# elybrand/quantized_neural_networks

Measured on AMD Instinct MI355X. Metric: weights_quantized_per_sec, higher is better.
Workload: dtype f64; 1 GPU; Dense(4096->4096) whole-layer GPFQ, m=1024 calibration samples, M=3 alphabet, alphabet_scalar=3 (BASELINE.json configs[1], the north-star layer); N=4096, C=4096, m=1024, M=3, neurons_per_gpu=4096, arithmetic=f32 products / f64 residual and dot products (reference's mixed flow)

## Files before the change

### quantized_neural_networks_amd/csrc/gpfq_blk.hip

```cpp
#include <atomic>
#include <cmath>
#include <cstring>
#include <type_traits>

#include <cstdlib>
#include <mutex>
#include "gpfq_device.hpp"
#include <hip/hip_ext.h>
#include "gpfq_launch.hpp"
#include "gpfq_roles.hpp"

namespace gpfq {

namespace {

struct BlkStats {
    double rden, G, cb, ca, Ea, nrm;
    double sE1, sE2;
};
struct BandEntry {
    double H1, H2, E1, E2;
};
static_assert(sizeof(BlkStats) == 64 && sizeof(BandEntry) == 32, "header layout");

// ... 433 lines not shown
template <int S, int NSW> struct BlkSplit { static constexpr const int *pw = PairSplit<S>::pw; };
template <> struct BlkSplit<4, 4>   { static constexpr int pw_[4] = {1, 1, 1, 1}; static constexpr const int *pw = pw_; };
template <> struct BlkSplit<32, 11> { static constexpr int pw_[11] = {3, 3, 3, 3, 3, 3, 3, 2, 3, 3, 3}; static constexpr const int *pw = pw_; };
template <> struct BlkSplit<24, 11> { static constexpr int pw_[11] = {2, 2, 2, 2, 2, 2, 2, 1, 3, 3, 3}; static constexpr const int *pw = pw_; };

template <> struct BlkSplit<64, 11> { static constexpr int pw_[11] = {4, 6, 6, 6, 6, 6, 6, 6, 6, 6, 6}; static constexpr const int *pw = pw_; };
template <> struct BlkSplit<48, 11> { static constexpr int pw_[11] = {4, 5, 4, 4, 5, 4, 4, 5, 4, 4, 5}; static constexpr const int *pw = pw_; };
template <> struct BlkSplit<16, 11> { static constexpr int pw_[11] = {2, 2, 1, 1, 2, 2, 1, 1, 1, 1, 2}; static constexpr const int *pw = pw_; };

struct BlkSplitQuad32 { static constexpr int pw[8] = {2, 5, 5, 4, 2, 5, 5, 4}; };
struct BlkSplitFour16 { static constexpr int pw[8] = {1, 2, 2, 3, 2, 2, 2, 2}; };
template <int S> struct BlkSplit7;
template <> struct BlkSplit7<32> { static constexpr int pw[7] = {5, 5, 5, 2, 5, 5, 5}; };
template <> struct BlkSplit7<24> { static constexpr int pw[7] = {4, 4, 4, 1, 4, 4, 3}; };
template <> struct BlkSplit7<16> { static constexpr int pw[7] = {3, 3, 2, 1, 3, 2, 2}; };
template <int G, int S, int NSW, int NL> constexpr const int *blk_split()
{
    if constexpr (NSW == 7) return BlkSplit7<S>::pw;
    else
    if constexpr (G == 4 && NL < 4 && S == 32 && NSW == 8) return BlkSplitQuad32::pw;
    else if constexpr (G == 1 && NL == 4 && S == 16 && NSW == 8) return BlkSplitFour16::pw;
    else return BlkSplit<S, NSW>::pw;
}

template <int G, int S, int NSW, int NL> constexpr bool blk_split_has(int k)
{
    for (int w = 0; w < NSW; ++w)
        if (blk_split<G, S, NSW, NL>()[w] == k) return true;
    return false;
}

template <int G, int PW, int MP, int B, int NSW, bool SYM, int NL, int CLM>
// ... 1 lines not shown
{
    constexpr bool CL = CLM != 0;
    constexpr int NB = NL * G, KQ = 64 / G, NW = blk_slots(NSW, NB);
    constexpr int RSH = NL == 4 ? 0 : (NL == 2 ? 1 : 2);
    constexpr int HDR = blk_hdr_bytes(B, CL);
    constexpr int RB = (int)blk_rec_bytes(MP, B, G, CL);
    lchar *lds = (lchar *)lds_generic;
    const int ng = lane & (G - 1), kq = lane / G, row = lane >> 4;
    const bool writer = (lane & 15 & ~(G - 1)) == 0 && (row & ((1 << RSH) - 1)) == 0;
    const int nloc = NL * ng;
    const int nrow = row >> RSH;
    const int64_t jbase = cs.cl * NB;
    const unsigned ldsT_addr = lds_addr(lds_generic), ldsW_addr = lds_addr(lds_generic + L.off_w);
    const int64_t N = K.N;
    const int nslots = K.nblk + 1;
    const int o_x  = HDR + 8 * (pbase + kq);
    int o_q = o_x + 4 * MP;
    asm volatile("" : "+v"(o_q));
    constexpr int DB = blk_row64(G, B) ? 16 : 8;
    const int o_d  = HDR + 8 * MP + DB * (pbase + kq);
    using DRaw = std::conditional_t<blk_row64(G, B), double2, float2>;
    auto ld_d = [&](int off) -> DRaw { return lds_ld<DRaw>(lds, off); };
    auto to_d2 = [](const DRaw &v) -> double2 { return make_double2((double)v.x, (double)v.y); };
    const int o_wq = L.off_wq + nloc * B * 8;
    const int o_dw = L.off_d + (wave * B * NB + nloc + nrow) * 8;
    const int o_x2 = L.off_x2 + (wave * NB + nloc + nrow) * 16;

    double u[NL][2 * PW];
#pragma unroll
    for (int i = 0; i < NL; ++i)
#pragma unroll
        for (int e = 0; e < 2 * PW; ++e) u[i][e] = 0.0;

    constexpr int NPIECES = (B * RB + 1023) >> 10;
    constexpr int PER_MIN = NPIECES / NSW;
// ... 18 lines not shown
    constexpr int NHP = (B * HDR + 1023) >> 10;
    auto load_headers = [&](int b2, int buf) {
        if (wave < NHP && b2 <= K.nblk)
            glds16_s(K.hdrs + (int64_t)b2 * B * HDR + ((int64_t)wave << 10), lane16,
                     lds_addr(lds_generic + L.off_hr) + (unsigned)buf * (unsigned)L.hr_pitch + ((unsigned)wave << 10));
    };
    for (int k = 0; wave + NSW * k < NPIECES; ++k) issue_piece(0, k);
    load_weights(0);
    load_headers(0, 0); load_headers(1, 1);
    dma_wait();
    slot_barrier();
    int hbuf = 2;
    unsigned long long st0 = 0, st1 = 0, st2 = 0, st3 = 0, st4 = 0, st5 = 0, acc_dma = 0, acc_u = 0, acc_d = 0, acc_w = 0, acc_b = 0, acc_t = 0;
    (void)st0; (void)st1; (void)st2; (void)st3; (void)st4; (void)st5; (void)acc_dma; (void)acc_u; (void)acc_d; (void)acc_w; (void)acc_b; (void)acc_t;

    constexpr bool kMfmaD = G == 4 && B == 4 && blk_row64(G, B) && !kNoMfmaD;
    constexpr bool kFused = kMfmaD && !kNoFused;
    constexpr bool kBatchTop = kFused && NL == 4 && NSW == 11;
    constexpr bool kTopSym = kBatchTop && SYM;
    constexpr bool kLateHdr = kTopSym && PW >= 2 && (kTop3 & 1) != 0, kLateW = kTopSym && PW >= 2 && (kTop3 & 2) != 0;
    constexpr int kHdrStep = PW >= 3 ? 8 : 6, kWStep = PW >= 3 ? 10 : 7;
    static_assert(!(kLateHdr || kLateW) || (PW <= 3 && B == 4 && PTS == 2 && PER_MIN <= 6), "the free pair-steps of a two- or three-pair wavefront");
    static_assert(!kLateW || NB * B == 64, "one 256-byte weight piece per block");
    unsigned long long w_lanes = 0ull, w_tail = 0ull;
    int w_whole = 0;
    const float *wsrc = nullptr;
    if constexpr (kLateW) {
        w_lanes = wave == 0 ? __builtin_amdgcn_ballot_w64(jbase + lane / B < K.C) : 0ull;
        w_tail = w_lanes & (0x1111111111111111ull * ((1ull << (int)(N % B)) - 1ull));
        w_whole = (int)(N / B);
        wsrc = K.Wt + (jbase + lane / B) * K.ldw + (int64_t)(B + lane % B) * K.ldt;
    }
    (void)w_lanes; (void)w_tail; (void)w_whole; (void)wsrc;
    constexpr bool kPreloadAll = PW * B <= 8 && PW <= 5 && !kFused;
    constexpr bool kHoist = kPreloadAll && PW * B <= 4;
    constexpr int PB = kPreloadAll ? B : 1, PP = kPreloadAll ? PW : 1;
    constexpr bool kPreD = kHoist && PW * B * (blk_row64(G, B) ? 4 : 2) <= 16 && !kMfmaD;
// ... 27 lines not shown
            const int nb_ = ((b + 1) & 1) * L.tile_pitch;
            const int cbq = (b & 1) * NB * B * 8;
            double eu[NL], ew[NL];
#pragma unroll
            for (int n = 0; n < NL; ++n) { eu[n] = 0.0; ew[n] = 0.0; }
#pragma unroll
            for (int n = 0; n < NL; ++n) {
                const float w = lds_ld<float2>(lds, o_wq + cbq + (n * B + S) * 8).x;
#pragma unroll 1
                for (int p = 0; p < PW; ++p) {
                    double t0 = u[n][0], t1 = u[n][1];
#pragma unroll
                    for (int pp = 1; pp < PW; ++pp) { t0 = (p == pp) ? u[n][2 * pp] : t0; t1 = (p == pp) ? u[n][2 * pp + 1] : t1; }
                    for (int j = 0; j < S; ++j) {
                        const int rb = nb_ + j * RB;
                        const float2 x2 = lds_ld<float2>(lds, rb + o_x + 8 * p * KQ), q2 = lds_ld<float2>(lds, rb + o_q + 8 * p * KQ);
                        const float2 wq = lds_ld<float2>(lds, o_wq + cbq + (n * B + j) * 8);
                        if constexpr (SYM) {
                            t0 += (double)__fmaf_rn(wq.y, q2.x, __fmul_rn(wq.x, x2.x));
                            t1 += (double)__fmaf_rn(wq.y, q2.y, __fmul_rn(wq.x, x2.y));
                        } else {
                            t0 += (double)__fsub_rn(__fmul_rn(wq.x, x2.x), __fmul_rn(wq.y, q2.x));
                            t1 += (double)__fsub_rn(__fmul_rn(wq.x, x2.y), __fmul_rn(wq.y, q2.y));
                        }
                    }
                    const int rb = nb_ + S * RB;
                    const float2 x2 = lds_ld<float2>(lds, rb + o_x + 8 * p * KQ);
                    float2 q2;
                    if constexpr (SYM) {
                        const int i0 = 2 * (pbase + p * KQ + kq);
                        const float *xr = K.Xq + ((int64_t)b * B + S) * K.ldx + (CL ? (int64_t)cs.slice * MP : (int64_t)0);
                        const int mrow = CL ? cs.m_sl : K.m;
                        q2.x = i0 < mrow ? xr[i0] : 0.f;
                        q2.y = i0 + 1 < mrow ? xr[i0 + 1] : 0.f;
                    } else {
                        q2 = lds_ld<float2>(lds, rb + o_q + 8 * p * KQ);
                    }
                    eu[n] = fma((double)q2.x, t0, eu[n]);
                    eu[n] = fma((double)q2.y, t1, eu[n]);
                    ew[n] = fma((double)q2.x, t0 + (double)__fmul_rn(w, x2.x), ew[n]);
                    ew[n] = fma((double)q2.y, t1 + (double)__fmul_rn(w, x2.y), ew[n]);
                }
            }
            const double vu = fold_klanes_n<G, NL>(eu), vw = fold_klanes_n<G, NL>(ew);
            if (writer) lds_st<double2>(lds, o_x2, make_double2(vu, vw));
            slot_barrier();
            slot_barrier();
            if constexpr (kBatchTop) ctl = lds_read_now(lds + L.off_ctl + 4 * (b & 1));
            else ctl = lds_ld<int>(lds, L.off_ctl + 4 * (b & 1));
        }
    };
// ... 27 lines not shown
            for (int n = 0; n < NL; ++n) pr[n] = pk2{wv[n], wv[n]} * xv;
            if constexpr (SYM) {
#pragma unroll
                for (int n = 0; n < NL; ++n) dd[n] = __builtin_elementwise_fma(pk2{qv[n], qv[n]}, qx, pr[n]);
            } else {
#pragma unroll
                for (int n = 0; n < NL; ++n) rr[n] = pk2{qv[n], qv[n]} * qx;
#pragma unroll
                for (int n = 0; n < NL; ++n) dd[n] = pr[n] - rr[n];
            }
#pragma unroll
            for (int n = 0; n < NL; ++n) { c0[n] = (double)dd[n].x; c1[n] = (double)dd[n].y; }
#pragma unroll
            for (int n = 0; n < NL; ++n) { u[n][2 * p] += c0[n]; u[n][2 * p + 1] += c1[n]; }
        };
        if constexpr (kFused) {
            const int rbm = tbase + ng * RB + o_d;
            constexpr int PF = NSW == 7 ? 2 : 1, NPS = PW * B;
            float2 fwq[B][NL], xbuf[PF], qbuf[PF];
            double2 dcur;
            auto row_off = [&](int i, bool q) { return tbase + (i % B) * RB + (q ? o_q : o_x) + 8 * (i / B) * KQ; };
            auto first_requests = [&]() {
#pragma unroll
                for (int s = 0; s < B; ++s)
#pragma unroll
                    for (int n = 0; n < NL; ++n) fwq[s][n] = lds_ld<float2>(lds, o_wq + pbq + (n * B + s) * 8);
#pragma unroll
                for (int i = 0; i < PF; ++i)
                    if (i < NPS) { xbuf[i] = lds_ld<float2>(lds, row_off(i, false)); qbuf[i] = lds_ld<float2>(lds, row_off(i, true)); }
                dcur = lds_ld<double2>(lds, rbm);
            };
            if constexpr (kTopSym) {
                static_assert(!kTopSym || (B == 4 && NL == 4 && PF == 1), "slot_top_sym: four neurons per lane, pair-steps 0..2 are pair 0's steps 0..2");
                nf4 w01[4], w23[4];
                nf2 x2n, q2n;
                nd2 d0;
                __builtin_amdgcn_s_setprio(2);
                slot_top_sym<RB>(w01, w23, x2n, q2n, d0, u[0][0], u[0][1], u[1][0], u[1][1], u[2][0], u[2][1], u[3][0], u[3][1],
                                 lds + row_off(0, false), lds + row_off(0, true), lds + o_wq + pbq, lds + rbm);
                __builtin_amdgcn_s_waitcnt(0xC07F);
                xbuf[0] = make_float2(x2n.x, x2n.y); qbuf[0] = make_float2(q2n.x, q2n.y);
                dcur = make_double2(d0.x, d0.y);
#pragma unroll
                for (int n = 0; n < NL; ++n) {
                    fwq[0][n] = make_float2(w01[n].x, w01[n].y); fwq[1][n] = make_float2(w01[n].z, w01[n].w);
                    fwq[2][n] = make_float2(w23[n].x, w23[n].y); fwq[3][n] = make_float2(w23[n].z, w23[n].w);
                }
// ... 1 lines not shown
                static_assert(!kBatchTop || (B == 4 && NL == 4), "lds_read_slot_top reads four neurons' steps 0 and 1: 16 bytes at a stride of 4 steps x 8 bytes");
                nf2 x0, q0;
                nf4 w01[4];
                lds_read_slot_top(x0, q0, w01, lds + row_off(0, false), lds + row_off(0, true), lds + o_wq + pbq);
                xbuf[0] = make_float2(x0.x, x0.y); qbuf[0] = make_float2(q0.x, q0.y);
#pragma unroll
                for (int n = 0; n < NL; ++n) { fwq[0][n] = make_float2(w01[n].x, w01[n].y); fwq[1][n] = make_float2(w01[n].z, w01[n].w); }
#pragma unroll
                for (int s = 2; s < B; ++s)
#pragma unroll
                    for (int n = 0; n < NL; ++n) fwq[s][n] = lds_ld<float2>(lds, o_wq + pbq + (n * B + s) * 8);
                dcur = lds_ld<double2>(lds, rbm);
            } else {
                first_requests();
            }
            double2 dprev = make_double2(0.0, 0.0);
            double acc[NL];
#pragma unroll
            for (int n = 0; n < NL; ++n) acc[n] = 0.0;
            auto mfma_pair = [&](int pp, int i, const double2 &dd) {
                const int n = i % NL, e = i / NL;
                acc[n] = __builtin_amdgcn_mfma_f64_4x4x4f64(u[n][2 * pp + e], e ? dd.y : dd.x, acc[n], 0, 0, 0);
            };
#pragma unroll
            for (int p = 0; p < PW; ++p) {
                {
                    const int pr = 2 - (3 * p) / PW;
                    if (p == 0 || pr != 2 - (3 * (p - 1)) / PW) {
                        const int v = pr;
                        if (v >= 2) __builtin_amdgcn_s_setprio(2);
                        else if (v == 1) __builtin_amdgcn_s_setprio(1);
                        else __builtin_amdgcn_s_setprio(0);
                    }
                }
                if (p > 0) dcur = lds_ld<double2>(lds, rbm + DB * p * KQ);
#pragma unroll
                for (int st = 0; st < B; ++st) {
                    const int ips = p * B + st;
                    if (kTopSym && ips < 2) continue;
                    const float2 x2 = xbuf[ips % PF], q2 = qbuf[ips % PF];
                    const int pn = (ips + 1) / B, sn = (ips + 1) % B;
                    (void)pn; (void)sn;
                    if (ips + PF < NPS) {
                        xbuf[ips % PF] = lds_ld<float2>(lds, row_off(ips + PF, false));
                        qbuf[ips % PF] = lds_ld<float2>(lds, row_off(ips + PF, true));
                    }
                    if (kTopSym && ips < 4) {
#pragma unroll
                        for (int i = 0; i < PPP; ++i) {
                            const int k = (PTS * (ips - 2)) * PPP + i;
                            if (PTS * B * PPP <= PER_MIN || k < PER_MIN) issue_piece(bn, k);
                        }
                    }
                    if (p < PTS) {
#pragma unroll
                        for (int i = 0; i < PPP; ++i) {
                            const int k = (PTS * st + p) * PPP + i;
                            if (PTS * B * PPP <= PER_MIN || k < PER_MIN) issue_piece(bn, k);
                        }
                    }
// ... 3 lines not shown
                        const unsigned on = ((unsigned)(wave - NHP) & (unsigned)(b2 - K.nblk - 1)) >> 31;
                        glds16_s_lanes(K.hdrs + (int64_t)b2 * B * HDR + ((int64_t)wave << 10), lane16,
                                       lds_addr(lds_generic + L.off_hr) + (unsigned)hbuf * (unsigned)L.hr_pitch + ((unsigned)wave << 10), 0ull - (unsigned long long)on);
                        hbuf = hbuf == 2 ? 0 : hbuf + 1;
                    }
                    if (kLateW && ips == kWStep) {
                        int b1 = b + 1;
                        asm volatile("" : "+s"(b1));
                        glds4_lanes(wsrc, ldsW_addr + (unsigned)((b1 & 1) * NB * B * 4), b1 < w_whole ? w_lanes : b1 == w_whole ? w_tail : 0ull);
                        wsrc += (int64_t)B * K.ldt;
                    }
                    __builtin_amdgcn_sched_barrier(0);
                    float wv[NL], qv[NL];
#pragma unroll
                    for (int n = 0; n < NL; ++n) { wv[n] = fwq[st][n].x; qv[n] = fwq[st][n].y; }
                    update_pair(p, x2, q2, wv, qv);
                    if (p > 0) {
#pragma unroll
                        for (int i = 0; i < 2 * NL; ++i)
                            if (i * B / (2 * NL) == st) mfma_pair(p - 1, i, dprev);
                    }
                    __builtin_amdgcn_sched_barrier(0);
                }
                dprev = dcur;
            }
            for (int k = PTS * B * PPP < PER_MIN ? PTS * B * PPP : PER_MIN; wave + NSW * k < NPIECES; ++k) issue_piece(bn, k);
            STAMP(st2);
#pragma unroll
            for (int i = 0; i < 2 * NL; ++i) mfma_pair(PW - 1, i, dprev);
#pragma unroll
            for (int n = 0; n < NL; ++n) { acc[n] = ror_add<8>(acc[n]); acc[n] = ror_add<4>(acc[n]); }
            if (b + 1 < nslots && (lane & 12) == 0) {
                const int od = L.off_d + ((((((b + 1) & 1) * NW + wave) * B) + (lane & 3)) * NB + NL * (lane >> 4)) * 8;
                if constexpr (NL == 4) {
                    lds_st<double2>(lds, od, make_double2(acc[0], acc[1]));
                    lds_st<double2>(lds, od + 16, make_double2(acc[2], acc[3]));
                } else if constexpr (NL == 2) {
                    lds_st<double2>(lds, od, make_double2(acc[0], acc[NL - 1]));
                } else {
                    lds_st<double>(lds, od, acc[0]);
                }
            }
        } else {
        if constexpr (kPreloadAll) {
            if constexpr (!kHoist) { preload_wq(b); preload_rows(b); __builtin_amdgcn_sched_barrier(0); }
#pragma unroll
            for (int s = 0; s < B; ++s) {
                if (s == 0) __builtin_amdgcn_s_setprio(2);
// ... 154 lines not shown
            if constexpr (kHoist) {
                if (b + 1 < nslots) { preload_wq(b + 1); preload_rows(b + 1); }
            }
        }
        }
    }

    STAMP_DO(
    if (K.stamps && blockIdx.x == 0 && lane == 0 && (wave == 0 || wave == 7)) {
        unsigned long long *o = K.stamps + (wave == 0 ? 0 : 8);
        o[0] = acc_dma; o[1] = acc_u; o[2] = acc_d; o[3] = acc_w; o[4] = acc_b; o[5] = (unsigned long long)nslots; o[6] = acc_t;
    }
    if (K.stamps && blockIdx.x == 0 && lane == 0) K.stamps[32 + wave] = acc_dma + acc_u + acc_d + acc_w;

    )
    if (K.resid) {
        double ss[NL];
#pragma unroll
        for (int n = 0; n < NL; ++n) {
            double q = 0.0;
#pragma unroll
            for (int e = 0; e < 2 * PW; ++e) q = fma(u[n][e], u[n][e], q);
            ss[n] = q;
        }
        const double v = fold_klanes_n<G, NL>(ss);
        if (writer) lds_st<double>(lds, o_dw, v);
    }
    slot_barrier();
    if (K.u_out) {
#pragma unroll
        for (int n = 0; n < NL; ++n) {
            const int64_t jn = jbase + nloc + n;
            if (jn < K.C) {
#pragma unroll
                for (int p = 0; p < PW; ++p)
#pragma unroll
                    for (int e = 0; e < 2; ++e) {
                        const int i = 2 * (pbase + p * KQ + kq) + e;
                        if constexpr (CL) {
                            if (i < cs.m_sl) K.u_out[jn * K.u_ld + (int64_t)cs.slice * MP + i] = u[n][2 * p + e];
                        } else {
                            if (i < K.m) K.u_out[jn * (int64_t)K.m + i] = u[n][2 * p + e];
                        }
                    }
            }
        }
    }
}

template <int G, int MP, int B, int NSW, bool SYM, int NL, int CLM, bool KOUT = false>
__device__ __forceinline__ void blk_decision_role(const BlkK &K, char *lds_generic, const BlkLds &L, int lane, ClState &cs)
{
    constexpr bool CL = CLM != 0;
// ... 745 lines not shown
    const bool four = C <= 1024 && opt.blk_four_groups;
    if (four && m > 768 && m <= 1024) return {1, 8, 4, 1024, 8, 4};
    if (four && m > 1024 && m <= 1536) return {1, 12, 2, 1536, 8, 4};
    if (four && m > 1536 && m <= 2048) return {1, 16, 2, 2048, 8, 4};
    if (m > 768 && m <= 1024) return C <= 2048 ? BlkShape{2, 16, 4, 1024, 8, 4} : BlkShape{4, 32, 4, 1024, nw4_long, 4};
    const int64_t rounds16 = (C + 4095) / 4096, rounds8 = (C + 2047) / 2048;
    const bool wide = C > 2048 && 8 * rounds16 <= 5 * rounds8 && opt.blk_wide_groups;
    if (m > 1024 && m <= 1536) return wide ? BlkShape{4, 48, 2, 1536, 11, 4} : BlkShape{2, 24, 2, 1536, 8, 4};
    if (m > 1536 && m <= 2048) return wide ? BlkShape{4, 64, 2, 2048, 11, 4} : BlkShape{2, 32, 2, 2048, 8, 4};
    if (m > 2048 && m <= 3072) return four ? BlkShape{1, 24, 1, 3072, 8, 4} : BlkShape{2, 48, 1, 3072, 11, 4};
    if (m > 3072 && m <= 4096) return four ? BlkShape{1, 32, 1, 4096, 8, 4} : BlkShape{2, 64, 1, 4096, 11, 4};
    if (m > 4096 && m <= 5120) return {1, 40, 1, 5120, 8, 4};
    return {0, 0, 0, 0, 0, 0};
}


__global__ void gpfq_alphabet_store_kernel(DevAlphabet *out, DevAlphabet D, unsigned *counters)
{
    if (threadIdx.x == 0 && blockIdx.x == 0) *out = D;
    if (counters && threadIdx.x < 16) counters[threadIdx.x] = 0u;
}

__global__ void gpfq_alphabet_device_kernel(DevAlphabet *out, const float *__restrict__ median32, double alphabet_scalar, AlphabetArg unit, int want_sym)
{
    if (threadIdx.x != 0 || blockIdx.x != 0) return;
    form_device_alphabet(out, median32[0], alphabet_scalar, unit, want_sym);
}

static size_t blk_recs_bytes(int64_t nblk, const BlkShape &sh)
{
// ... 34 lines not shown
        const BlkShape sh = blk_shape(m, C, opt);
        if (!sh.G) continue;
        const int64_t nblk = (N + sh.B - 1) / sh.B;
        const size_t b = blk_recs_bytes(nblk, sh) * (size_t)(sh.NS ? sh.NS : 1) + ((blk_hdrs_bytes(nblk, sh.B, sh.NS != 0) + 255) & ~(size_t)255) + blk_mbox_bytes(Cn, sh);
        if (b > need) need = b;
    }
    return need ? need + kAlphaBlock : 0;
}

static float blk_sym_a(const PipeArgs &a)
{
    if ((a.opt.variant >> 4) & 2) return 0.f;
    return blk_sym_of(a.A.a, a.A.M);
}

constexpr bool blk_kout_shape(int G, int B, int NL, int CLM) { return G == 4 && B == 4 && NL == 4 && CLM == 0; }

template <int G, int S, int B, int NSW, bool SYM, int NL, int CLM = 0, bool KOUT = false>
static hipError_t launch_blk_sym(const PipeArgs &a, const BlkShape &sh, const DevAlphabet *alpha, hipStream_t stream)
{
    constexpr bool CL = CLM != 0;
    if constexpr (!KOUT && blk_kout_shape(G, B, NL, CLM)) {
        if (a.o_st != 1) return launch_blk_sym<G, S, B, NSW, SYM, NL, CLM, true>(a, sh, alpha, stream);
    }
    if (!KOUT && a.o_st != 1) return hipErrorInvalidValue;
    constexpr int NB = NL * G;
    const BlkLds L = blk_lds(sh.mp, NB, B, NSW, G, CL);
    const unsigned grid = CL ? (unsigned)(blk_clusters(a.C, sh) * sh.NS) : (unsigned)((a.C + NB - 1) / NB);
    auto *kern = gpfq_blk_kernel<G, S, B, NSW, SYM, NL, CLM, KOUT>;
    hipError_t e = ensure_dynamic_lds((const void *)kern, (size_t)L.total);
    if (e != hipSuccess) return e;
// ... 141 lines not shown
            hipLaunchKernelGGL((gpfq_blk_prep_kernel<4, true, true>), dim3((unsigned)nrec), dim3(256), 0, stream, a.X, a.Xq, a.ld, a.N, (int)a.m, sh.mp * sh.NS,
                               nrm32, wbase, wbase + blk_hdrs_off(nblk, sh), alpha, sym_prep,
                               sh.NS, (int64_t)blk_recs_bytes(nblk, sh));
            e = hipGetLastError();
            if (e != hipSuccess) return e;
        }
        if (!do_run) return hipSuccess;
        ClusterLaunchGuard one_at_a_time(stream);
        if (one_at_a_time.err != hipSuccess) return one_at_a_time.err;
#define GPFQ_BLK_CL(S_, NSW_, NL_, M_) (sym ? launch_blk_sym<4, S_, 4, NSW_, true, NL_, M_>(a, sh, alpha, stream) : launch_blk_sym<4, S_, 4, NSW_, false, NL_, M_>(a, sh, alpha, stream))
        if (sh.S == 24) {
            const int forced = a.opt.blk_cluster768;
            const int nw = forced == 8 || forced == 11 ? forced : (sym ? 11 : 8);
            return nw == 8 ? GPFQ_BLK_CL(24, 8, 4, 1) : GPFQ_BLK_CL(24, 11, 4, 1);
        }
        if (sh.NL == 4) return GPFQ_BLK_CL(32, 11, 4, 1);
        return sh.NL == 1 ? GPFQ_BLK_CL(32, 8, 1, 1) : GPFQ_BLK_CL(32, 8, 2, 1);
#undef GPFQ_BLK_CL
    }
    auto *prep = sh.B == 4 ? (r64 ? gpfq_blk_prep_kernel<4, true> : gpfq_blk_prep_kernel<4, false>)
                           : (sh.B == 2 ? (r64 ? gpfq_blk_prep_kernel<2, true> : gpfq_blk_prep_kernel<2, false>) : gpfq_blk_prep_kernel<1, false>);
    const int sym = sym_prep;
    if (!do_prep) {
    } else if (run_form) {
        int run = 8;
        if (prep_run >= 4 && prep_run <= kPrepRunMax) run = prep_run;
        else {
            int64_t best = -1;
            for (int rl = 4; rl <= kPrepRunMax; ++rl) {
                const int64_t wgs = (nrec + rl - 1) / rl, cost = ((wgs + 1023) / 1024) * (1 + rl);
// ... 30 lines not shown
        if (sh.B == 4) return sh.S == 4 ? launch_blk_inst<1, 4, 4, 4, 2>(a, sh, alpha, stream) : launch_blk_inst<1, 8, 4, 8, 2>(a, sh, alpha, stream);
        if (sh.B == 2) return sh.S == 12 ? launch_blk_inst<1, 12, 2, 8, 2>(a, sh, alpha, stream) : launch_blk_inst<1, 16, 2, 8, 2>(a, sh, alpha, stream);
        if (sh.S == 24) return launch_blk_inst<1, 24, 1, 8, 2>(a, sh, alpha, stream);
        return sh.S == 32 ? launch_blk_inst<1, 32, 1, 8, 2>(a, sh, alpha, stream) : launch_blk_inst<1, 40, 1, 8, 2>(a, sh, alpha, stream);
    }
    if (sh.B == 1 && sh.S == 40) return launch_blk_inst<1, 40, 1>(a, sh, alpha, stream);
    if (sh.B == 1) {
        if (sh.G == 2) return sh.S == 64 ? launch_blk_inst<2, 64, 1, 11>(a, sh, alpha, stream) : launch_blk_inst<2, 48, 1, 11>(a, sh, alpha, stream);
        return sh.S == 32 ? launch_blk_inst<1, 32, 1>(a, sh, alpha, stream) : launch_blk_inst<1, 24, 1>(a, sh, alpha, stream);
    }
    if (sh.G == 4 && sh.S == 64) return launch_blk_inst<4, 64, 2, 11>(a, sh, alpha, stream);
    if (sh.G == 4 && sh.S == 48) return launch_blk_inst<4, 48, 2, 11>(a, sh, alpha, stream);
    if (sh.G == 4 && sh.NW == 11) {
        if (sh.S == 16) return launch_blk_inst<4, 16, 4, 11>(a, sh, alpha, stream);
        if (sh.S == 24) return launch_blk_inst<4, 24, 4, 11>(a, sh, alpha, stream);
        return launch_blk_inst<4, 32, 4, 11>(a, sh, alpha, stream);
    }
    if (sh.G == 4) {
        if (sh.S == 16) return launch_blk_inst<4, 16, 4>(a, sh, alpha, stream);
        if (sh.S == 24) return launch_blk_inst<4, 24, 4>(a, sh, alpha, stream);
        return launch_blk_inst<4, 32, 4>(a, sh, alpha, stream);
    }
    if (sh.G == 1) {
        if (sh.S == 8) return launch_blk_inst<1, 8, 4>(a, sh, alpha, stream);
        if (sh.S == 12) return launch_blk_inst<1, 12, 2>(a, sh, alpha, stream);
        return launch_blk_inst<1, 16, 2>(a, sh, alpha, stream);
    }
    if (sh.B == 4) return launch_blk_inst<2, 16, 4>(a, sh, alpha, stream);
    if (sh.S == 24) return launch_blk_inst<2, 24, 2>(a, sh, alpha, stream);
    return launch_blk_inst<2, 32, 2>(a, sh, alpha, stream);
// ... 4 lines not shown
```

### quantized_neural_networks_amd/csrc/gpfq_options.hpp

```cpp
#pragma once

namespace gpfq {

#define GPFQ_OPTIONS(X)                                                                                                                      \
                                                                                      \
    X(onchip_mode, 1, true, v ? 1 : 0, "")                                                                \
    X(tile_steps, 0, v >= 0 && v <= 64 && !(v & (v - 1)), v, "0 or a power of two <= 64")                                 \
    X(group_waves, 0, v >= 0 && v <= 16, v, "in [0, 16]")                                                                 \
    X(lanes_per_neuron, 0, v == 0 || v == 1 || v == 16 || v == 32 || v == 64, v, "0, 1, 16, 32 or 64")    \
    X(waves_per_neuron, 0, v >= 0 && v <= 16, v, "in [0, 16]")   \
    X(variant, 0, true, v, "")                                   \
    X(pipe, -1, v >= -1 && v <= 2, v, "-1, 0, 1 or 2")           \
    X(auto_gram, 1, true, v ? 1 : 0, "")                         \
    X(gram_slack_log2, 0, true, v, "")                           \
    X(sync_errors, 0, true, v ? 1 : 0, "")                       \
                                                              \
    X(blk_single_groups, 1, true, v ? 1 : 0, "")                                   \
    X(blk_pair_groups, 1, true, v ? 1 : 0, "")                                     \
    X(blk_four_groups, 1, true, v ? 1 : 0, "")                   \
    X(blk_wide_groups, 1, true, v ? 1 : 0, "")                   \
    X(blk_quad_groups, 2, true, v < 0 ? 0 : (v > 2 ? 2 : v), "")    \
    X(blk_quad_waves, 0, v == 0 || v == 7 || v == 8, v, "0 (by shape), 7 or 8")       \
    X(blk_sweep_waves, 0, v == 0 || v == 8 || v == 11, v, "0 (by shape), 8 or 11")    \
    X(blk_prep_run, 1, true, v >= 4 && v <= 16 ? v : (v ? 1 : 0), "")    \
    X(blk_prep_norms, 1, true, v ? 1 : 0, "")                    \
                                    \
    X(blk_cluster, 1, v == 0 || v == 1 || v >= 1024, v, "0 (off), 1 (default: by row length and width) or a row length >= 1024")    \
    X(blk_cluster_nl, 0, true, v == 1 || v == 2 || v == 4 ? v : 0, "")    \
    X(blk_cluster_map, -1, true, v < 0 ? -1 : (v ? 1 : 0), "")   \
    X(blk_cluster768, -1, true, v == 0 || v == 8 || v == 11 ? v : -1, "")    \
    X(blk_chip_ok, -1, true, v < 0 ? -1 : (v ? 1 : 0), "")       \
    X(blk_cluster_timeout_ms, 3000, v >= 1 && v <= 60000, v, "in [1, 60000]")    \
    X(blk_cluster_fault, 0, true, v ? 1 : 0, "")                 \
                                                                                                                            \
    X(conv_fused, 1, true, v ? 1 : 0, "")                        \
    X(conv_planes_free, 1, true, v ? 1 : 0, "")                  \
    X(conv_nhwc, 1, true, v ? 1 : 0, "")                         \
    X(conv_strip, 0, v == 0 || v == 1 || v == 2 || v == 4, v, "0, 1, 2 or 4")    \
// ... 15 lines not shown
```

### quantized_neural_networks_amd/csrc/gpfq_roles.hpp

```cpp
#pragma once

#include "gpfq_device.hpp"

namespace gpfq {
namespace {

constexpr int kSweepWaves = 8;

template <int ROR>
__device__ __forceinline__ double ror_add(double x)
{
    const int lo = __builtin_amdgcn_mov_dpp(__double2loint(x), 0x120 + ROR, 0xF, 0xF, true);
    const int hi = __builtin_amdgcn_mov_dpp(__double2hiint(x), 0x120 + ROR, 0xF, 0xF, true);
    return x + __hiloint2double(hi, lo);
}

__device__ __forceinline__ double fold32(double x, double y)
{
    const auto lo = __builtin_amdgcn_permlane32_swap((unsigned)__double2loint(x), (unsigned)__double2loint(y), false, false);
    const auto hi = __builtin_amdgcn_permlane32_swap((unsigned)__double2hiint(x), (unsigned)__double2hiint(y), false, false);
    return __hiloint2double((int)hi[0], (int)lo[0]) + __hiloint2double((int)hi[1], (int)lo[1]);
}

__device__ __forceinline__ double fold16(double x, double y)
// ... 224 lines not shown
                 "s_waitcnt lgkmcnt(7)\n\tv_pk_mul_f32 v[152:153], v[164:165], v[36:37] op_sel_hi:[1,0]\n\t"
                 "v_pk_mul_f32 v[154:155], v[164:165], v[32:33] op_sel_hi:[1,0]\n\t"
                 "v_pk_mul_f32 v[156:157], v[164:165], v[28:29] op_sel_hi:[1,0]\n\t"
                 "v_pk_mul_f32 v[164:165], v[164:165], v[24:25] op_sel_hi:[1,0]\n\t"
                 GPFQ_TOP_PAIR_STEP("v[36:37]", "v[32:33]", "v[28:29]", "v[24:25]", "v[164:165]", "v164", "v165", "v[166:167]")
                 "s_waitcnt lgkmcnt(0)"
                 : "=&{v[34:37]}"(w01[0]), "=&{v[30:33]}"(w01[1]), "=&{v[26:29]}"(w01[2]), "=&{v[22:25]}"(w01[3]),
                   [w2] "=&v"(w23[0]), [w3] "=&v"(w23[1]), [w4] "=&v"(w23[2]), [w5] "=&v"(w23[3]), [d] "=&v"(d), [x2] "=&v"(x2), [q2] "=&v"(q2),
                   [u00] "+v"(u00), [u01] "+v"(u01), [u10] "+v"(u10), [u11] "+v"(u11), [u20] "+v"(u20), [u21] "+v"(u21), [u30] "+v"(u30), [u31] "+v"(u31)
                 : [ax] "v"((unsigned)(uintptr_t)px), [aq] "v"((unsigned)(uintptr_t)pq), [aw] "v"((unsigned)(uintptr_t)pwq), [ad] "v"((unsigned)(uintptr_t)pd),
                   [r1] "i"(RB), [r2] "i"(2 * RB)
                 : "memory", "v148", "v149", "v150", "v151", "v152", "v153", "v154", "v155", "v156", "v157", "v158", "v159", "v160", "v161", "v162",
                   "v163", "v164", "v165", "v166", "v167");
#undef GPFQ_TOP_PAIR_STEP
}
__device__ __forceinline__ int lds_read_now(lchar *p)
{
    int v;
    asm volatile("ds_read_b32 %0, %1\n\ts_waitcnt lgkmcnt(0)" : "=&v"(v) : "v"((unsigned)(uintptr_t)p) : "memory");
    return v;
}

}
}
```

Before: 5.998 billion weights/s.

## Add eight-group lane map with two neurons per lane for symmetric blk sweep

```diff
diff --git a/quantized_neural_networks_amd/csrc/gpfq_blk.hip b/quantized_neural_networks_amd/csrc/gpfq_blk.hip
--- a/quantized_neural_networks_amd/csrc/gpfq_blk.hip
+++ b/quantized_neural_networks_amd/csrc/gpfq_blk.hip
@@ -471,8 +471,11 @@
 template <> struct BlkSplit7<32> { static constexpr int pw[7] = {5, 5, 5, 2, 5, 5, 5}; };
 template <> struct BlkSplit7<24> { static constexpr int pw[7] = {4, 4, 4, 1, 4, 4, 3}; };
 template <> struct BlkSplit7<16> { static constexpr int pw[7] = {3, 3, 2, 1, 3, 2, 2}; };
+struct BlkSplitOct64 { static constexpr int pw[11] = {6, 6, 6, 6, 6, 6, 6, 4, 6, 6, 6}; };
 template <int G, int S, int NSW, int NL> constexpr const int *blk_split()
 {
+    if constexpr (G == 8) { static_assert(S == 64 && NSW == 11 && NL == 2, "the eight-group map: 1024-sample rows over eleven sweep wavefronts"); return BlkSplitOct64::pw; }
+    else
     if constexpr (NSW == 7) return BlkSplit7<S>::pw;
     else
     if constexpr (G == 4 && NL < 4 && S == 32 && NSW == 8) return BlkSplitQuad32::pw;
@@ -504,11 +507,14 @@
     const unsigned ldsT_addr = lds_addr(lds_generic), ldsW_addr = lds_addr(lds_generic + L.off_w);
     const int64_t N = K.N;
     const int nslots = K.nblk + 1;
-    const int o_x  = HDR + 8 * (pbase + kq);
+    constexpr int PU = G == 8 ? 2 : 1;
+    static_assert(PW % PU == 0, "whole units per wavefront");
+    auto pair_off = [](int p) { return PU * (p / PU) * KQ + p % PU; };
+    const int o_x  = HDR + 8 * (pbase + PU * kq);
     int o_q = o_x + 4 * MP;
     asm volatile("" : "+v"(o_q));
     constexpr int DB = blk_row64(G, B) ? 16 : 8;
-    const int o_d  = HDR + 8 * MP + DB * (pbase + kq);
+    const int o_d  = HDR + 8 * MP + DB * (pbase + PU * kq);
     using DRaw = std::conditional_t<blk_row64(G, B), double2, float2>;
     auto ld_d = [&](int off) -> DRaw { return lds_ld<DRaw>(lds, off); };
     auto to_d2 = [](const DRaw &v) -> double2 { return make_double2((double)v.x, (double)v.y); };
@@ -557,13 +563,15 @@
     unsigned long long st0 = 0, st1 = 0, st2 = 0, st3 = 0, st4 = 0, st5 = 0, acc_dma = 0, acc_u = 0, acc_d = 0, acc_w = 0, acc_b = 0, acc_t = 0;
     (void)st0; (void)st1; (void)st2; (void)st3; (void)st4; (void)st5; (void)acc_dma; (void)acc_u; (void)acc_d; (void)acc_w; (void)acc_b; (void)acc_t;
 
-    constexpr bool kMfmaD = G == 4 && B == 4 && blk_row64(G, B) && !kNoMfmaD;
-    constexpr bool kFused = kMfmaD && !kNoFused;
-    constexpr bool kBatchTop = kFused && NL == 4 && NSW == 11;
+    constexpr bool kMfmaD = (G == 4 || (G == 8 && NL == 2)) && B == 4 && blk_row64(G, B) && (!kNoMfmaD || G == 8);
+    constexpr bool kFused = kMfmaD && (!kNoFused || G == 8);
+    static_assert(G != 8 || kFused, "the eight-group lane map exists in the fused form only");
+    constexpr bool kBatchTop = kFused && (NL == 4 || G == 8) && NSW == 11;
     constexpr bool kTopSym = kBatchTop && SYM;
-    constexpr bool kLateHdr = kTopSym && PW >= 2 && (kTop3 & 1) != 0, kLateW = kTopSym && PW >= 2 && (kTop3 & 2) != 0;
-    constexpr int kHdrStep = PW >= 3 ? 8 : 6, kWStep = PW >= 3 ? 10 : 7;
-    static_assert(!(kLateHdr || kLateW) || (PW <= 3 && B == 4 && PTS == 2 && PER_MIN <= 6), "the free pair-steps of a two- or three-pair wavefront");
+    constexpr int NUW = PW / PU;
+    constexpr bool kLateHdr = kTopSym && NUW >= 2 && (kTop3 & 1) != 0, kLateW = kTopSym && NUW >= 2 && (kTop3 & 2) != 0;
+    constexpr int kHdrStep = NUW >= 3 ? 8 : 6, kWStep = NUW >= 3 ? 10 : 7;
+    static_assert(!(kLateHdr || kLateW) || (NUW <= 3 && B == 4 && PTS == 2 && PER_MIN <= 6), "the free pair-steps of a two- or three-pair wavefront");
     static_assert(!kLateW || NB * B == 64, "one 256-byte weight piece per block");
     unsigned long long w_lanes = 0ull, w_tail = 0ull;
     int w_whole = 0;
@@ -621,7 +629,7 @@
                     for (int pp = 1; pp < PW; ++pp) { t0 = (p == pp) ? u[n][2 * pp] : t0; t1 = (p == pp) ? u[n][2 * pp + 1] : t1; }
                     for (int j = 0; j < S; ++j) {
                         const int rb = nb_ + j * RB;
-                        const float2 x2 = lds_ld<float2>(lds, rb + o_x + 8 * p * KQ), q2 = lds_ld<float2>(lds, rb + o_q + 8 * p * KQ);
+                        const float2 x2 = lds_ld<float2>(lds, rb + o_x + 8 * pair_off(p)), q2 = lds_ld<float2>(lds, rb + o_q + 8 * pair_off(p));
                         const float2 wq = lds_ld<float2>(lds, o_wq + cbq + (n * B + j) * 8);
                         if constexpr (SYM) {
                             t0 += (double)__fmaf_rn(wq.y, q2.x, __fmul_rn(wq.x, x2.x));
@@ -632,16 +640,16 @@
                         }
                     }
                     const int rb = nb_ + S * RB;
-                    const float2 x2 = lds_ld<float2>(lds, rb + o_x + 8 * p * KQ);
+                    const float2 x2 = lds_ld<float2>(lds, rb + o_x + 8 * pair_off(p));
                     float2 q2;
                     if constexpr (SYM) {
-                        const int i0 = 2 * (pbase + p * KQ + kq);
+                        const int i0 = 2 * (pbase + pair_off(p) + PU * kq);
                         const float *xr = K.Xq + ((int64_t)b * B + S) * K.ldx + (CL ? (int64_t)cs.slice * MP : (int64_t)0);
                         const int mrow = CL ? cs.m_sl : K.m;
                         q2.x = i0 < mrow ? xr[i0] : 0.f;
                         q2.y = i0 + 1 < mrow ? xr[i0 + 1] : 0.f;
                     } else {
-                        q2 = lds_ld<float2>(lds, rb + o_q + 8 * p * KQ);
+                        q2 = lds_ld<float2>(lds, rb + o_q + 8 * pair_off(p));
                     }
                     eu[n] = fma((double)q2.x, t0, eu[n]);
                     eu[n] = fma((double)q2.y, t1, eu[n]);
@@ -699,12 +707,55 @@
 #pragma unroll
             for (int n = 0; n < NL; ++n) { u[n][2 * p] += c0[n]; u[n][2 * p + 1] += c1[n]; }
         };
+        auto update_unit2 = [&](int P, const float4 &x4, const float4 &q4, const float (&wv)[NL], const float (&qv)[NL]) {
+            const pk2 xv[2] = {{x4.x, x4.y}, {x4.z, x4.w}}, qx[2] = {{q4.x, q4.y}, {q4.z, q4.w}};
+            pk2 pr[2][NL], rr[2][NL], dd[2][NL];
+            double c0[2][NL], c1[2][NL];
+#pragma unroll
+            for (int h = 0; h < 2; ++h)
+#pragma unroll
+                for (int n = 0; n < NL; ++n) pr[h][n] = pk2{wv[n], wv[n]} * xv[h];
+            if constexpr (SYM) {
+#pragma unroll
+                for (int h = 0; h < 2; ++h)
+#pragma unroll
+                    for (int n = 0; n < NL; ++n) dd[h][n] = __builtin_elementwise_fma(pk2{qv[n], qv[n]}, qx[h], pr[h][n]);
+            } else {
+#pragma unroll
+                for (int h = 0; h < 2; ++h)
+#pragma unroll
+                    for (int n = 0; n < NL; ++n) rr[h][n] = pk2{qv[n], qv[n]} * qx[h];
+#pragma unroll
+                for (int h = 0; h < 2; ++h)
+#pragma unroll
+                    for (int n = 0; n < NL; ++n) dd[h][n] = pr[h][n] - rr[h][n];
+            }
+#pragma unroll
+            for (int h = 0; h < 2; ++h)
+#pragma unroll
+                for (int n = 0; n < NL; ++n) { c0[h][n] = (double)dd[h][n].x; c1[h][n] = (double)dd[h][n].y; }
+#pragma unroll
+            for (int h = 0; h < 2; ++h)
+#pragma unroll
+                for (int n = 0; n < NL; ++n) { u[n][4 * P + 2 * h] += c0[h][n]; u[n][4 * P + 2 * h + 1] += c1[h][n]; }
+        };
+        (void)update_unit2;
         if constexpr (kFused) {
-            const int rbm = tbase + ng * RB + o_d;
-            constexpr int PF = NSW == 7 ? 2 : 1, NPS = PW * B;
-            float2 fwq[B][NL], xbuf[PF], qbuf[PF];
-            double2 dcur;
-            auto row_off = [&](int i, bool q) { return tbase + (i % B) * RB + (q ? o_q : o_x) + 8 * (i / B) * KQ; };
+            const int rbm = tbase + (G == 8 ? lane & 3 : ng) * RB + o_d;
+            constexpr int NU = PW / PU;
+            constexpr int PF = NSW == 7 ? 2 : 1, NPS = NU * B;
+            using XRow = std::conditional_t<PU == 2, float4, float2>;
+            struct DRow2 { double2 v[2]; };
+            using DRow = std::conditional_t<PU == 2, DRow2, double2>;
+            auto dhalf = [](const DRow &r, int h) -> const double2 & { if constexpr (PU == 2) return r.v[h]; else return r; };
+            float2 fwq[B][NL];
+            XRow xbuf[PF], qbuf[PF];
+            DRow dcur;
+            auto row_off = [&](int i, bool q) { return tbase + (i % B) * RB + (q ? o_q : o_x) + 8 * PU * (i / B) * KQ; };
+            auto ld_drow = [&](int off) -> DRow {
+                if constexpr (PU == 2) return DRow{{lds_ld<double2>(lds, off), lds_ld<double2>(lds, off + 16)}};
+                else return lds_ld<double2>(lds, off);
+            };
             auto first_requests = [&]() {
 #pragma unroll
                 for (int s = 0; s < B; ++s)
@@ -712,10 +763,26 @@
                     for (int n = 0; n < NL; ++n) fwq[s][n] = lds_ld<float2>(lds, o_wq + pbq + (n * B + s) * 8);
 #pragma unroll
                 for (int i = 0; i < PF; ++i)
-                    if (i < NPS) { xbuf[i] = lds_ld<float2>(lds, row_off(i, false)); qbuf[i] = lds_ld<float2>(lds, row_off(i, true)); }
-                dcur = lds_ld<double2>(lds, rbm);
+                    if (i < NPS) { xbuf[i] = lds_ld<XRow>(lds, row_off(i, false)); qbuf[i] = lds_ld<XRow>(lds, row_off(i, true)); }
+                dcur = ld_drow(rbm);
             };
-            if constexpr (kTopSym) {
+            if constexpr (kTopSym && G == 8) {
+                static_assert(!(kTopSym && G == 8) || (B == 4 && NL == 2 && PU == 2 && PF == 1), "slot_top_sym2: two neurons per lane, pair-steps 0..2 are unit 0's steps 0..2");
+                nf4 w01[2], w23[2], x2n, q2n;
+                nd2 d01[2];
+                __builtin_amdgcn_s_setprio(2);
+                slot_top_sym2<RB>(w01, w23, x2n, q2n, d01, u[0][0], u[0][1], u[0][2], u[0][3], u[1][0], u[1][1], u[1][2], u[1][3],
+                                  lds + row_off(0, false), lds + row_off(0, true), lds + o_wq + pbq, lds + rbm);
+                __builtin_amdgcn_s_waitcnt(0xC07F);
+                __builtin_memcpy(&xbuf[0], &x2n, sizeof(XRow)); __builtin_memcpy(&qbuf[0], &q2n, sizeof(XRow));
+#pragma unroll
+                for (int h = 0; h < PU; ++h) dcur.v[h] = make_double2(d01[h].x, d01[h].y);
+#pragma unroll
+                for (int n = 0; n < NL; ++n) {
+                    fwq[0][n] = make_float2(w01[n].x, w01[n].y); fwq[1][n] = make_float2(w01[n].z, w01[n].w);
+                    fwq[2][n] = make_float2(w23[n].x, w23[n].y); fwq[3][n] = make_float2(w23[n].z, w23[n].w);
+                }
+            } else if constexpr (kTopSym) {
                 static_assert(!kTopSym || (B == 4 && NL == 4 && PF == 1), "slot_top_sym: four neurons per lane, pair-steps 0..2 are pair 0's steps 0..2");
                 nf4 w01[4], w23[4];
                 nf2 x2n, q2n;
@@ -747,36 +814,40 @@
             } else {
                 first_requests();
             }
-            double2 dprev = make_double2(0.0, 0.0);
+            DRow dprev;
+            if constexpr (PU == 2) dprev = DRow{{make_double2(0.0, 0.0), make_double2(0.0, 0.0)}};
+            else dprev = make_double2(0.0, 0.0);
             double acc[NL];
 #pragma unroll
             for (int n = 0; n < NL; ++n) acc[n] = 0.0;
-            auto mfma_pair = [&](int pp, int i, const double2 &dd) {
+            constexpr int NM = 2 * PU * NL;
+            auto mfma_pair = [&](int pp, int i, const DRow &dd) {
                 const int n = i % NL, e = i / NL;
-                acc[n] = __builtin_amdgcn_mfma_f64_4x4x4f64(u[n][2 * pp + e], e ? dd.y : dd.x, acc[n], 0, 0, 0);
+                const double2 &dh = dhalf(dd, e / 2);
+                acc[n] = __builtin_amdgcn_mfma_f64_4x4x4f64(u[n][2 * PU * pp + e], (e & 1) ? dh.y : dh.x, acc[n], 0, 0, 0);
             };
 #pragma unroll
-            for (int p = 0; p < PW; ++p) {
+            for (int p = 0; p < NU; ++p) {
                 {
-                    const int pr = 2 - (3 * p) / PW;
-                    if (p == 0 || pr != 2 - (3 * (p - 1)) / PW) {
+                    const int pr = 2 - (3 * p) / NU;
+                    if (p == 0 || pr != 2 - (3 * (p - 1)) / NU) {
                         const int v = pr;
                         if (v >= 2) __builtin_amdgcn_s_setprio(2);
                         else if (v == 1) __builtin_amdgcn_s_setprio(1);
                         else __builtin_amdgcn_s_setprio(0);
                     }
                 }
-                if (p > 0) dcur = lds_ld<double2>(lds, rbm + DB * p * KQ);
+                if (p > 0) dcur = ld_drow(rbm + DB * PU * p * KQ);
 #pragma unroll
                 for (int st = 0; st < B; ++st) {
                     const int ips = p * B + st;
                     if (kTopSym && ips < 2) continue;
-                    const float2 x2 = xbuf[ips % PF], q2 = qbuf[ips % PF];
+                    const XRow x2 = xbuf[ips % PF], q2 = qbuf[ips % PF];
                     const int pn = (ips + 1) / B, sn = (ips + 1) % B;
                     (void)pn; (void)sn;
                     if (ips + PF < NPS) {
-                        xbuf[ips % PF] = lds_ld<float2>(lds, row_off(ips + PF, false));
-                        qbuf[ips % PF] = lds_ld<float2>(lds, row_off(ips + PF, true));
+                        xbuf[ips % PF] = lds_ld<XRow>(lds, row_off(ips + PF, false));
+                        qbuf[ips % PF] = lds_ld<XRow>(lds, row_off(ips + PF, true));
                     }
                     if (kTopSym && ips < 4) {
 #pragma unroll
@@ -810,11 +881,12 @@
                     float wv[NL], qv[NL];
 #pragma unroll
                     for (int n = 0; n < NL; ++n) { wv[n] = fwq[st][n].x; qv[n] = fwq[st][n].y; }
-                    update_pair(p, x2, q2, wv, qv);
+                    if constexpr (PU == 2) update_unit2(p, x2, q2, wv, qv);
+                    else update_pair(p, x2, q2, wv, qv);
                     if (p > 0) {
 #pragma unroll
-                        for (int i = 0; i < 2 * NL; ++i)
-                            if (i * B / (2 * NL) == st) mfma_pair(p - 1, i, dprev);
+                        for (int i = 0; i < NM; ++i)
+                            if (i * B / NM == st) mfma_pair(p - 1, i, dprev);
                     }
                     __builtin_amdgcn_sched_barrier(0);
                 }
@@ -823,11 +895,16 @@
             for (int k = PTS * B * PPP < PER_MIN ? PTS * B * PPP : PER_MIN; wave + NSW * k < NPIECES; ++k) issue_piece(bn, k);
             STAMP(st2);
 #pragma unroll
-            for (int i = 0; i < 2 * NL; ++i) mfma_pair(PW - 1, i, dprev);
-#pragma unroll
-            for (int n = 0; n < NL; ++n) { acc[n] = ror_add<8>(acc[n]); acc[n] = ror_add<4>(acc[n]); }
-            if (b + 1 < nslots && (lane & 12) == 0) {
-                const int od = L.off_d + ((((((b + 1) & 1) * NW + wave) * B) + (lane & 3)) * NB + NL * (lane >> 4)) * 8;
+            for (int i = 0; i < NM; ++i) mfma_pair(NU - 1, i, dprev);
+#pragma unroll
+            for (int n = 0; n < NL; ++n) {
+                acc[n] = ror_add<8>(acc[n]);
+                if constexpr (G == 4) acc[n] = ror_add<4>(acc[n]);
+            }
+            const bool dwriter = G == 8 ? (lane & 8) == 0 : (lane & 12) == 0;
+            const int dgroup = G == 8 ? (lane >> 4) + (lane & 4) : lane >> 4;
+            if (b + 1 < nslots && dwriter) {
+                const int od = L.off_d + ((((((b + 1) & 1) * NW + wave) * B) + (lane & 3)) * NB + NL * dgroup) * 8;
                 if constexpr (NL == 4) {
                     lds_st<double2>(lds, od, make_double2(acc[0], acc[1]));
                     lds_st<double2>(lds, od + 16, make_double2(acc[2], acc[3]));
@@ -1012,6 +1089,25 @@
     if (K.stamps && blockIdx.x == 0 && lane == 0) K.stamps[32 + wave] = acc_dma + acc_u + acc_d + acc_w;
 
     )
+    if constexpr (G == 8) {
+        if (K.resid) {
+            double ss[4];
+#pragma unroll
+            for (int n = 0; n < NL; ++n)
+#pragma unroll
+                for (int h = 0; h < PU; ++h) {
+                    double q = 0.0;
+#pragma unroll
+                    for (int P = 0; P < PW / PU; ++P)
+#pragma unroll
+                        for (int e = 0; e < 2; ++e) q = fma(u[n][2 * (PU * P + h) + e], u[n][2 * (PU * P + h) + e], q);
+                    ss[PU * n + h] = q;
+                }
+            double v = fold_klanes<G>(ss);
+            v = fold16(v, v);
+            if (writer) lds_st<double>(lds, o_dw, v);
+        }
+    } else
     if (K.resid) {
         double ss[NL];
 #pragma unroll
@@ -1034,7 +1130,7 @@
                 for (int p = 0; p < PW; ++p)
 #pragma unroll
                     for (int e = 0; e < 2; ++e) {
-                        const int i = 2 * (pbase + p * KQ + kq) + e;
+                        const int i = 2 * (pbase + pair_off(p) + PU * kq) + e;
                         if constexpr (CL) {
                             if (i < cs.m_sl) K.u_out[jn * K.u_ld + (int64_t)cs.slice * MP + i] = u[n][2 * p + e];
                         } else {
@@ -1810,6 +1906,14 @@
     return {0, 0, 0, 0, 0, 0};
 }
 
+constexpr int kGroupsByShape = 8;
+static int blk_groups(const BlkShape &sh, bool sym, const Options &opt)
+{
+    const bool applies = sym && sh.G == 4 && sh.S == 32 && sh.B == 4 && sh.NW == 11 && sh.NL == 4;
+    if (!applies) return 4;
+    return opt.blk_groups ? opt.blk_groups : kGroupsByShape;
+}
+
 
 __global__ void gpfq_alphabet_store_kernel(DevAlphabet *out, DevAlphabet D, unsigned *counters)
 {
@@ -1874,7 +1978,7 @@
     return blk_sym_of(a.A.a, a.A.M);
 }
 
-constexpr bool blk_kout_shape(int G, int B, int NL, int CLM) { return G == 4 && B == 4 && NL == 4 && CLM == 0; }
+constexpr bool blk_kout_shape(int G, int B, int NL, int CLM) { return ((G == 4 && NL == 4) || (G == 8 && NL == 2)) && B == 4 && CLM == 0; }
 
 template <int G, int S, int B, int NSW, bool SYM, int NL, int CLM = 0, bool KOUT = false>
 static hipError_t launch_blk_sym(const PipeArgs &a, const BlkShape &sh, const DevAlphabet *alpha, hipStream_t stream)
@@ -2046,6 +2150,10 @@
             const int nw = forced == 8 || forced == 11 ? forced : (sym ? 11 : 8);
             return nw == 8 ? GPFQ_BLK_CL(24, 8, 4, 1) : GPFQ_BLK_CL(24, 11, 4, 1);
         }
+        if (sh.NL == 4 && blk_groups(sh, sym != 0, a.opt) == 8) {
+            note_dense_kernel("gpfq_blk_kernel, cluster form (rows cut into 1024-sample slices: one workgroup of 11 sweep wavefronts + 1 decision wavefront per slice, partial dot products exchanged once per slot; eight neuron groups)");
+            return launch_blk_sym<8, 64, 4, 11, true, 2, 1>(a, sh, alpha, stream);
+        }
         if (sh.NL == 4) return GPFQ_BLK_CL(32, 11, 4, 1);
         return sh.NL == 1 ? GPFQ_BLK_CL(32, 8, 1, 1) : GPFQ_BLK_CL(32, 8, 2, 1);
 #undef GPFQ_BLK_CL
@@ -2106,6 +2214,10 @@
     if (sh.G == 4 && sh.NW == 11) {
         if (sh.S == 16) return launch_blk_inst<4, 16, 4, 11>(a, sh, alpha, stream);
         if (sh.S == 24) return launch_blk_inst<4, 24, 4, 11>(a, sh, alpha, stream);
+        if (blk_groups(sh, sym_shape != 0, a.opt) == 8) {
+            note_dense_kernel("gpfq_blk_kernel (4 to 11 sweep wavefronts + 1 decision wavefront per workgroup, blocks of steps per slot; eight neuron groups)");
+            return launch_blk_sym<8, 64, 4, 11, true, 2>(a, sh, alpha, stream);
+        }
         return launch_blk_inst<4, 32, 4, 11>(a, sh, alpha, stream);
     }
     if (sh.G == 4) {
diff --git a/quantized_neural_networks_amd/csrc/gpfq_options.hpp b/quantized_neural_networks_amd/csrc/gpfq_options.hpp
--- a/quantized_neural_networks_amd/csrc/gpfq_options.hpp
+++ b/quantized_neural_networks_amd/csrc/gpfq_options.hpp
@@ -22,6 +22,7 @@
     X(blk_quad_groups, 2, true, v < 0 ? 0 : (v > 2 ? 2 : v), "")    \
     X(blk_quad_waves, 0, v == 0 || v == 7 || v == 8, v, "0 (by shape), 7 or 8")       \
     X(blk_sweep_waves, 0, v == 0 || v == 8 || v == 11, v, "0 (by shape), 8 or 11")    \
+    X(blk_groups, 0, v == 0 || v == 4 || v == 8, v, "0 (by shape), 4 or 8")             \
     X(blk_prep_run, 1, true, v >= 4 && v <= 16 ? v : (v ? 1 : 0), "")    \
     X(blk_prep_norms, 1, true, v ? 1 : 0, "")                    \
                                     \
diff --git a/quantized_neural_networks_amd/csrc/gpfq_roles.hpp b/quantized_neural_networks_amd/csrc/gpfq_roles.hpp
--- a/quantized_neural_networks_amd/csrc/gpfq_roles.hpp
+++ b/quantized_neural_networks_amd/csrc/gpfq_roles.hpp
@@ -262,6 +262,51 @@
                    "v163", "v164", "v165", "v166", "v167");
 #undef GPFQ_TOP_PAIR_STEP
 }
+template <int RB>
+__device__ __forceinline__ void slot_top_sym2(nf4 (&w01)[2], nf4 (&w23)[2], nf4 &x2, nf4 &q2, nd2 (&d)[2],
+                                              double &u00, double &u01, double &u02, double &u03, double &u10, double &u11, double &u12, double &u13,
+                                              lchar *px, lchar *pq, lchar *pwq, lchar *pd)
+{
+    static_assert(2 * RB + 16 <= 65536, "the rows of pair-steps 1 and 2 are reached through the 16-bit offset field");
+#define GPFQ_TOP2_PAIR_STEP(W0, W1, XA, XAL, XAH, XB, XBL, XBH, QA, QB)                                            \
+    "v_pk_fma_f32 v[160:161], " W0 ", " QA ", v[160:161] op_sel:[1,0,0]\n\t"                                       \
+    "v_pk_fma_f32 v[162:163], " W0 ", " QB ", v[162:163] op_sel:[1,0,0]\n\t"                                       \
+    "v_pk_fma_f32 " XA ", " W1 ", " QA ", " XA " op_sel:[1,0,0]\n\t"                                               \
+    "v_pk_fma_f32 " XB ", " W1 ", " QB ", " XB " op_sel:[1,0,0]\n\t"                                               \
+    "v_cvt_f64_f32 " QA ", v160\n\tv_cvt_f64_f32 v[160:161], v161\n\t"                                             \
+    "v_cvt_f64_f32 v[164:165], " XAL "\n\tv_cvt_f64_f32 " XA ", " XAH "\n\t"                                       \
+    "v_cvt_f64_f32 " QB ", v162\n\tv_cvt_f64_f32 v[162:163], v163\n\t"                                             \
+    "v_cvt_f64_f32 v[166:167], " XBL "\n\tv_cvt_f64_f32 " XB ", " XBH "\n\t"                                       \
+    "v_add_f64 %[u01], %[u01], v[160:161]\n\tv_add_f64 %[u10], %[u10], v[164:165]\n\t"                             \
+    "v_add_f64 %[u11], %[u11], " XA "\n\tv_add_f64 %[u02], %[u02], " QB "\n\t"                                     \
+    "v_add_f64 %[u03], %[u03], v[162:163]\n\tv_add_f64 %[u12], %[u12], v[166:167]\n\t"                             \
+    "v_add_f64 %[u00], %[u00], " QA "\n\tv_add_f64 %[u13], %[u13], " XB "\n\t"
+    asm volatile("ds_read_b128 v[144:147], %[ax]\n\tds_read_b128 v[148:151], %[aq]\n\t"
+                 "ds_read_b128 v[26:29], %[aw]\n\tds_read_b128 v[22:25], %[aw] offset:32\n\t"
+                 "ds_read_b128 v[152:155], %[ax] offset:%[r1]\n\tds_read_b128 v[156:159], %[aq] offset:%[r1]\n\t"
+                 "ds_read_b128 %[w2], %[aw] offset:16\n\tds_read_b128 %[w3], %[aw] offset:48\n\t"
+                 "ds_read_b128 %[d0], %[ad]\n\tds_read_b128 %[d1], %[ad] offset:16\n\t"
+                 "ds_read_b128 %[x2], %[ax] offset:%[r2]\n\tds_read_b128 %[q2], %[aq] offset:%[r2]\n\t"
+                 "s_waitcnt lgkmcnt(9)\n\tv_pk_mul_f32 v[160:161], v[144:145], v[26:27] op_sel_hi:[1,0]\n\t"
+                 "v_pk_mul_f32 v[162:163], v[146:147], v[26:27] op_sel_hi:[1,0]\n\t"
+                 "s_waitcnt lgkmcnt(8)\n\tv_pk_mul_f32 v[144:145], v[144:145], v[22:23] op_sel_hi:[1,0]\n\t"
+                 "v_pk_mul_f32 v[146:147], v[146:147], v[22:23] op_sel_hi:[1,0]\n\t"
+                 GPFQ_TOP2_PAIR_STEP("v[26:27]", "v[22:23]", "v[144:145]", "v144", "v145", "v[146:147]", "v146", "v147", "v[148:149]", "v[150:151]")
+                 "s_waitcnt lgkmcnt(6)\n\tv_pk_mul_f32 v[160:161], v[152:153], v[28:29] op_sel_hi:[1,0]\n\t"
+                 "v_pk_mul_f32 v[162:163], v[154:155], v[28:29] op_sel_hi:[1,0]\n\t"
+                 "v_pk_mul_f32 v[152:153], v[152:153], v[24:25] op_sel_hi:[1,0]\n\t"
+                 "v_pk_mul_f32 v[154:155], v[154:155], v[24:25] op_sel_hi:[1,0]\n\t"
+                 GPFQ_TOP2_PAIR_STEP("v[28:29]", "v[24:25]", "v[152:153]", "v152", "v153", "v[154:155]", "v154", "v155", "v[156:157]", "v[158:159]")
+                 "s_waitcnt lgkmcnt(0)"
+                 : "=&{v[26:29]}"(w01[0]), "=&{v[22:25]}"(w01[1]), [w2] "=&v"(w23[0]), [w3] "=&v"(w23[1]), [d0] "=&v"(d[0]), [d1] "=&v"(d[1]),
+                   [x2] "=&v"(x2), [q2] "=&v"(q2),
+                   [u00] "+v"(u00), [u01] "+v"(u01), [u02] "+v"(u02), [u03] "+v"(u03), [u10] "+v"(u10), [u11] "+v"(u11), [u12] "+v"(u12), [u13] "+v"(u13)
+                 : [ax] "v"((unsigned)(uintptr_t)px), [aq] "v"((unsigned)(uintptr_t)pq), [aw] "v"((unsigned)(uintptr_t)pwq), [ad] "v"((unsigned)(uintptr_t)pd),
+                   [r1] "i"(RB), [r2] "i"(2 * RB)
+                 : "memory", "v144", "v145", "v146", "v147", "v148", "v149", "v150", "v151", "v152", "v153", "v154", "v155", "v156", "v157", "v158",
+                   "v159", "v160", "v161", "v162", "v163", "v164", "v165", "v166", "v167");
+#undef GPFQ_TOP2_PAIR_STEP
+}
 __device__ __forceinline__ int lds_read_now(lchar *p)
 {
     int v;
```

New measurement: 6.370 billion weights/s, median of 6. 6.2% higher.
